# tlepoint/fhe.rs

Measured on NVIDIA H100. Metric: bfv_ct_mul_relin_per_sec_n32768_14x62bit, higher is better.
Workload: dtype u64

## Files before the change

### fhe_rs_b200/csrc/capi.cu

```cuda
#include <algorithm>
#include <atomic>
#include <cstring>
#include <map>
#include <memory>
#include <mutex>
#include <string>
#include <vector>

#include "../../include/fhe_b200.h"
#include "engine.hpp"
#include "host/precompute.hpp"

using namespace fhe_b200;

namespace {

thread_local std::string g_last_error;

struct ScalerData {
  ScalerTablesH h;
  ScalerDev dev;
};

struct LevelData {
// ... 334 lines not shown
    FHE_CUDA(cudaEventRecord(ev[ns], user));
    for (u32 i = 0; i < ns; i++) FHE_CUDA(cudaStreamWaitEvent(par->side[i], ev[ns], 0));
  }
  template <class F>
  void run(F&& body) {
    u32 k = 0;
    for (u32 c0 = 0; c0 < count; c0 += chunk, k++) body(c0, std::min(chunk, count - c0), ns > 1 ? par->side[k % ns] : user);
    join();
  }
  void join() {
    if (ns < 2 || joined) return;
    joined = true;
    for (u32 i = 0; i < ns; i++)
      if (cudaEventRecord(ev[i], par->side[i]) == cudaSuccess) cudaStreamWaitEvent(user, ev[i], 0);
  }
  ~ChunkRunner() {
    join();
    for (cudaEvent_t e : ev)
      if (e) cudaEventDestroy(e);
  }
  bool joined = false;
};

void check_same(const fhe_b200_batch* a, const fhe_b200_batch* b) {
  if (a->par != b->par) throw FheError(FHE_B200_CONTEXT_MISMATCH, "ParameterMismatch: batches use different parameters");
  if (a->level != b->level) throw FheError(FHE_B200_INVALID_LEVEL, "InvalidLevel: operands are at different levels");
  if (a->mul_basis != b->mul_basis || a->limbs != b->limbs)
    throw FheError(FHE_B200_CONTEXT_MISMATCH, "PolynomialContextMismatch");
}
void need_repr(const fhe_b200_batch* b, int repr) {
  if (b->repr != repr) throw FheError(FHE_B200_INVALID_REPRESENTATION, "IncorrectRepresentation");
}
const RowIds& ids_of(const fhe_b200_batch* b) {
  const LevelData& lv = b->par->level(b->level);
  return b->mul_basis ? lv.mul_ids : lv.ctx_ids;
}

void key_switch_core(const fhe_b200_params* par, const fhe_b200_ksk* k, const u64* c2, u32 cts, const u64* base0,
                     const u64* base1, u64* out0, u64* out1, u32 out_ct_rows, Workspace& ws, cudaStream_t st) {
  const LevelData& kl = par->level(k->ksk_level);
  const u32 L = k->n_dig, Lk = k->Lk;
  u64* inter = ws.words(((size_t)cts * L * Lk) << par->logn);
  bool adjacent = false;
  if (k->log_base) {
    u64* dig = ws.words(((size_t)cts * L) << par->logn);
    launch_decompose(c2, dig, cts, L, k->log_base, par->logn, st);
    launch_ntt(dig, inter, cts * L, kl.ctx_ids, par->d_limbs, par->logn, false, 1, false, st, true);
  } else {
  u64 qmax = 0, qmin = ~0ull;
  for (u32 i = 0; i < L; i++) qmax = std::max(qmax, par->moduli[i]);
  for (u32 j = 0; j < Lk; j++) qmin = std::min(qmin, par->moduli[j]);
  const bool reduce = qmax > 4 * qmin - 1 || qmin < (1ull << 8);
  adjacent = Lk > 1 && ntt_uses_tma(cts * L * Lk, kl.ctx_ids, par->logn, Lk, c2, inter);
  launch_ntt(c2, inter, cts * L * Lk, kl.ctx_ids, par->d_limbs, par->logn, false, Lk, reduce, st, true, adjacent, L);
  }
  launch_ksmac(inter, k->k0, k->k1, base0, base1, out0, out1, cts, L, Lk, out_ct_rows, kl.ctx_ids, par->d_limbs,
               par->logn, st, adjacent);
}

void key_switch_apply(const fhe_b200_params* par, const fhe_b200_ksk* k, const u64* c2, u32 cts, u64* out,
                      int base_mode, u64* base, Workspace& ws, cudaStream_t st) {
  const LevelData& cl = par->level(k->ct_level);
  const u32 L = cl.L, Lk = k->Lk, logn = par->logn;
  const size_t row = (size_t)1 << logn;
  if (Lk == L) {
    const u64* b0 = base_mode == 1 ? out : base_mode == 2 ? base : nullptr;
    const u64* b1 = base_mode == 1 ? out + L * row : nullptr;
    key_switch_core(par, k, c2, cts, b0, b1, out, out + L * row, 2 * L, ws, st);
    return;
  }
  u64* cur = ws.words((size_t)cts * 2 * Lk * row);
  key_switch_core(par, k, c2, cts, nullptr, nullptr, cur, cur + Lk * row, 2 * Lk, ws, st);
  const LevelData& kl = par->level(k->ksk_level);
  launch_ntt(cur, cur, cts * 2 * Lk, kl.ctx_ids, par->d_limbs, logn, true, 1, false, st);
  for (u32 lv = k->ksk_level; lv < k->ct_level; lv++) {
    const LevelData& from = par->level(lv);
    u64* nxt = ws.words((size_t)cts * 2 * (from.L - 1) * row);
    launch_switch_down(from.sd, cur, nxt, cts * 2, from.L, from.ctx_ids, par->d_limbs, logn, st);
    cur = nxt;
  }
  launch_ntt(cur, cur, cts * 2 * L, cl.ctx_ids, par->d_limbs, logn, false, 1, false, st);
  if (base_mode == 1) {
    launch_ew(EW_ADD, out, cur, (size_t)cts * 2 * L, cl.ctx_ids, par->d_limbs, logn, st);
  } else {
    FHE_CUDA(cudaMemcpyAsync(out, cur, (size_t)cts * 2 * L * row * sizeof(u64), cudaMemcpyDeviceToDevice, st));
    if (base_mode == 2) {
      FHE_CUDA(cudaMemset2DAsync(base + L * row, 2 * L * row * sizeof(u64), 0, L * row * sizeof(u64), cts, st));
      launch_ew(EW_ADD, out, base, (size_t)cts * 2 * L, cl.ctx_ids, par->d_limbs, logn, st);
    }
  }
}

void mul_core(const fhe_b200_params* par, const LevelData& lv, const u64* a, const u64* b, u32 cts, u64* out0,
              u64* out1, int split, Workspace& ws, cudaStream_t st) {
  const u32 L = lv.L, E = lv.E, K = lv.K, logn = par->logn;
  const size_t row = (size_t)1 << logn;
  u64* A_l = ws.words((size_t)cts * 2 * L * row);
  u64* A_r = ws.words((size_t)cts * 2 * L * row);
  u64* X_l = ws.words((size_t)cts * 2 * E * row);
  u64* X_r = ws.words((size_t)cts * 2 * E * row);
  u64* T = ws.words((size_t)cts * 3 * K * row);
  RowIds ext_ids;
  std::memset(&ext_ids, 0, sizeof(ext_ids));
  ext_ids.limbs_per_poly = E;
  for (u32 j = 0; j < E; j++) ext_ids.ids[j] = lv.mul_ids.ids[L + j];
  launch_ntt(a, A_l, cts * 2 * L, lv.ctx_ids, par->d_limbs, logn, true, 1, false, st);
// ... 985 lines not shown
```

### fhe_rs_b200/csrc/engine.hpp

```cpp
#pragma once
#include <atomic>
#include <cuda_runtime.h>

#include "ntt.cuh"

namespace fhe_b200 {

extern std::atomic<unsigned long long> g_launches;

struct CudaFail {
  cudaError_t err;
  const char* what;
};
#define FHE_CUDA(x)                                         \
  do {                                                      \
    cudaError_t e__ = (x);                                  \
    if (e__ != cudaSuccess) throw CudaFail{e__, #x};        \
  } while (0)

void ensure_dynamic_smem(const void* kernel, size_t bytes);

struct RowIds {
  u32 limbs_per_poly;
  unsigned short ids[kMaxPos];
};

void launch_ntt(const u64* in, u64* out, u32 n_rows, const RowIds& ids, const LimbDev* limbs, u32 logn,
                bool inverse, u32 in_div, bool reduce_on_load, cudaStream_t st, bool lazy_out = false,
                bool digit_adjacent = false, u32 n_dig = 1);

bool launch_tensor_inverse_ntt(const u64* a, const u64* b, const u64* xa, const u64* xb, u64* T, u32 cts, u32 L, u32 K,
                               const RowIds& mul_ids, const LimbDev* limbs, u32 logn, cudaStream_t st);

enum EwOp { EW_ADD = 0, EW_SUB = 1, EW_NEG = 2 };
void launch_ew(EwOp op, u64* a, const u64* b, size_t n_rows, const RowIds& ids, const LimbDev* limbs, u32 logn,
               cudaStream_t st);

void launch_mul_plain(u64* a, const u64* pt, u32 cts, u32 parts, u32 n_pt, const RowIds& ids, const LimbDev* limbs,
                      u32 logn, cudaStream_t st, u32 op = 0);

void launch_dot(const u64* ct, const u64* pt, u64* out, u32 groups, u32 n_terms, u32 parts, u32 ct_count,
                u32 pt_count, const RowIds& ids, const LimbDev* limbs, u32 logn, cudaStream_t st);

void launch_tensor(const u64* a, const u64* b, const u64* xa, const u64* xb, u64* out, u32 cts, u32 L, u32 nca,
                   u32 ncb, u32 K, const RowIds& mul_ids, const LimbDev* limbs, u32 logn, cudaStream_t st);

void launch_tensor_nm(const u64* a, const u64* b, const u64* xa, const u64* xb, u64* out, u32 cts, u32 L, u32 E, u32 na,
                      u32 nb, const RowIds& mul_ids, const LimbDev* limbs, u32 logn, cudaStream_t st);

struct ScalerDev {
  u32 n_from, n_to, is_one, shift;
  u64 tg_lo, tg_hi;
  u32 tg_sign;
  u32 all_solinas;
  const u64* gamma;
  const u64* omega;
  const u64* to_lo;
  const u64* to_hi;
  const unsigned char* to_sign;
  const unsigned char* to_order;
  u32 n_pos, n_terms;
  const u64* tgar_lo;
  const u64* tgar_hi;
  unsigned short to_ids[kMaxPos];
};
void launch_scale(const ScalerDev& S, const LimbDev* limbs, const u64* in, u64* out0, u64* out1, u32 polys,
                  u32 out_rows_per_poly, u32 start, u32 n_out, int split3, u32 logn, cudaStream_t st);

void launch_ksmac(const u64* inter, const u64* k0, const u64* k1, const u64* base0, const u64* base1, u64* out0,
                  u64* out1, u32 cts, u32 n_dig, u32 Lk, u32 out_ct_rows, const RowIds& ids, const LimbDev* limbs,
                  u32 logn, cudaStream_t st, bool adjacent = false);

bool ntt_uses_tma(u32 n_rows, const RowIds& ids, u32 logn, u32 in_div, const u64* in, const u64* out);

void launch_decompose(const u64* in, u64* out, size_t polys, u32 n_dig, u32 log_base, u32 logn, cudaStream_t st);

void launch_gather(const u64* in, u64* out, size_t n_rows, const int* perm, u32 logn, cudaStream_t st);
void launch_substitute_power(const u64* in, u64* out, size_t n_rows, u32 exponent, const RowIds& ids,
                             const LimbDev* limbs, u32 logn, cudaStream_t st);

struct SwitchDownDev {
  u64 q_last, q_last_half;
  const u64* half_mod;
  const u64* inv;
  const u64* inv_s;
};
void launch_switch_down(const SwitchDownDev& S, const u64* in, u64* out, u32 polys, u32 L, const RowIds& ids,
                        const LimbDev* limbs, u32 logn, cudaStream_t st);

struct PackDev {
  u32 limbs;
  unsigned char nbits[kMaxPos];
  u32 offs[kMaxPos];
  u32 poly_bytes;
};
void launch_pack(const PackDev& P, const u64* words, unsigned char* bytes, size_t n_rows, u32 logn, cudaStream_t st);
void launch_unpack(const PackDev& P, const unsigned char* bytes, u64* words, size_t n_rows, u32 logn, cudaStream_t st);

}
```

### fhe_rs_b200/csrc/ntt.cu

```cuda
#include <algorithm>
#include <cstdint>
#include <cstdlib>
#include <cstring>
#include <map>
#include <mutex>
#include <utility>

#include "engine.hpp"
#include "ntt_fast.cuh"
#include "ntt_tma.cuh"

namespace fhe_b200 {

std::atomic<unsigned long long> g_launches{0};

void ensure_dynamic_smem(const void* kernel, size_t bytes) {
  if (bytes <= 48 * 1024) return;
  static std::mutex mu;
  static std::map<std::pair<int, const void*>, size_t> granted;
  int dev = 0;
  FHE_CUDA(cudaGetDevice(&dev));
  std::lock_guard<std::mutex> g(mu);
  size_t& have = granted[std::make_pair(dev, kernel)];
  if (have >= bytes) return;
// ... 171 lines not shown
  g_launches++;
}

template <bool INV>
void run_tma_rows(const u64* in, u64 in_rows, u64* out, u64 out_rows, const NttTmaArgs& A, cudaStream_t st) {
  static const int v = tma_variant("FHE_B200_TMA_ROWS", 2);
  if (v == 2 && A.n_polys % 2 == 0 && !(A.digit_adjacent && A.n_dig % 2)) {
    run_tma_rows_pair<INV, 3, 3>(in, in_rows, out, out_rows, A, st);
    return;
  }
  if (v == 26) run_tma_rows_v<INV, 2, 6>(in, in_rows, out, out_rows, A, st);
  else run_tma_rows_v<INV, 4, 4>(in, in_rows, out, out_rows, A, st);
}
template <int LOGP, bool INV, int STAGES, int MINB>
void run_tma_cols_v(const u64* in, u64 in_rows, u64* out, u64 out_rows, NttTmaArgs A, cudaStream_t st) {
  using Cfg = ColsCfg<LOGP, STAGES>;
  const CUtensorMap mi = cols_map(in, in_rows, A.logn, Cfg::BOX_ROWS), mo = cols_map(out, out_rows, A.logn, Cfg::BOX_ROWS);
  A.tiles_per_row = 4;
  A.tiles_total = A.lpp * 4 * A.n_polys;
  const u32 grid = std::min<u64>(A.tiles_total, (u64)sm_count() * MINB);
  if (!INV && A.reduce_on_load) {
    auto k = ntt_tma_cols_kernel<LOGP, INV, STAGES, MINB, !INV>;
    ensure_dynamic_smem((const void*)k, Cfg::SMEM);
    k<<<grid, Cfg::NT + 32, Cfg::SMEM, st>>>(mi, mo, A);
  } else {
    auto k = ntt_tma_cols_kernel<LOGP, INV, STAGES, MINB, false>;
    ensure_dynamic_smem((const void*)k, Cfg::SMEM);
    k<<<grid, Cfg::NT + 32, Cfg::SMEM, st>>>(mi, mo, A);
  }
  g_launches++;
}
template <int LOGP, bool INV>
void run_tma_cols(const u64* in, u64 in_rows, u64* out, u64 out_rows, const NttTmaArgs& A, cudaStream_t st) {
  static const int v = tma_variant("FHE_B200_TMA_COLS", 3);
  if (LOGP == 9) {
    if (v == 2) run_tma_cols_v<9, INV, 2, 1>(in, in_rows, out, out_rows, A, st);
    else run_tma_cols_v<9, INV, 3, 1>(in, in_rows, out, out_rows, A, st);
  } else if (LOGP == 8) {
    if (v == 2) run_tma_cols_v<8, INV, 2, 3>(in, in_rows, out, out_rows, A, st);
    else run_tma_cols_v<8, INV, 3, 2>(in, in_rows, out, out_rows, A, st);
  } else {
    if (v == 2) run_tma_cols_v<7, INV, 2, 6>(in, in_rows, out, out_rows, A, st);
    else run_tma_cols_v<7, INV, 3, 4>(in, in_rows, out, out_rows, A, st);
  }
}
template <bool INV>
void run_tma_cols_for(const u64* in, u64 in_rows, u64* out, u64 out_rows, const NttTmaArgs& A, cudaStream_t st) {
  switch (A.logn - 6) {
    case 7: run_tma_cols<7, INV>(in, in_rows, out, out_rows, A, st); break;
    case 8: run_tma_cols<8, INV>(in, in_rows, out, out_rows, A, st); break;
    case 9: run_tma_cols<9, INV>(in, in_rows, out, out_rows, A, st); break;
    default: throw TmaFail{};
  }
}

bool launch_ntt_tma(const u64* in, u64* out, u32 n_rows, const RowIds& ids, const LimbDev* limbs, u32 logn, bool inverse,
                    u32 in_div, bool reduce_on_load, cudaStream_t st, bool lazy_out, bool digit_adjacent, u32 n_dig) {
  const u32 lpp = ids.limbs_per_poly;
  if (logn < 13 || logn > 15 || !tensor_map_encoder()) return false;
  if (n_rows % lpp != 0 || (in_div != 1 && in_div != lpp)) return false;
  if (digit_adjacent && ((n_rows / lpp) % n_dig != 0 || n_dig == 0)) return false;
  if ((reinterpret_cast<uintptr_t>(in) | reinterpret_cast<uintptr_t>(out)) & 127) return false;
  NttTmaArgs A;
  std::memset(&A, 0, sizeof(A));
  A.limbs = limbs;
  A.n_polys = n_rows / lpp;
  A.lpp = lpp;
  A.logn = logn;
  A.digit_adjacent = digit_adjacent ? 1 : 0;
  A.n_dig = digit_adjacent ? n_dig : 1;
  for (int i = 0; i < kMaxPos; i++) A.ids[i] = ids.ids[i];
  const u64 in_rows = in_div == 1 ? n_rows : n_rows / lpp;
  try {
    NttTmaArgs first = A, second = A;
    first.in_bcast = in_div != 1;
    if (!inverse) {
      first.reduce_on_load = reduce_on_load;
      second.lazy_out = lazy_out;
      run_tma_cols_for<false>(in, in_rows, out, n_rows, first, st);
      run_tma_rows<false>(out, n_rows, out, n_rows, second, st);
    } else {
      if (reduce_on_load || in_div != 1) return false;
      run_tma_rows<true>(in, in_rows, out, n_rows, first, st);
      run_tma_cols_for<true>(out, n_rows, out, n_rows, second, st);
    }
  } catch (const TmaFail&) {
    return false;
  }
  return true;
}

template <int STAGES, int MINB>
void run_tensor_rows(const CUtensorMap& ma, const CUtensorMap& mb, const CUtensorMap& mxa, const CUtensorMap& mxb,
                     const CUtensorMap& mo, TensorRowsArgs A, cudaStream_t st) {
  using Cfg = TensorRowsCfg<kRowsRlog, STAGES>;
  auto k = ntt_tma_tensor_rows_kernel<kRowsRlog, STAGES, MINB>;
  ensure_dynamic_smem((const void*)k, Cfg::SMEM);
  const u32 grid = std::min<u64>(A.items_total, (u64)sm_count() * MINB);
  k<<<grid, Cfg::NT + 32, Cfg::SMEM, st>>>(ma, mb, mxa, mxb, mo, A);
  g_launches++;
}

bool launch_tensor_intt_tma(const u64* a, const u64* b, const u64* xa, const u64* xb, u64* T, u32 cts, u32 L, u32 K,
                            const RowIds& mul_ids, const LimbDev* limbs, u32 logn, cudaStream_t st) {
  constexpr u32 R = 1u << kRowsRlog;
  const u32 E = K - L;
  try {
    const CUtensorMap ma = rows_map(a, (u64)cts * 2 * L, logn, 4 * R), mb = rows_map(b, (u64)cts * 2 * L, logn, 4 * R);
    const CUtensorMap mxa = rows_map(xa, (u64)cts * 2 * E, logn, 4 * R), mxb = rows_map(xb, (u64)cts * 2 * E, logn, 4 * R);
    const CUtensorMap mo = rows_map(T, (u64)cts * 3 * K, logn, 4 * R);
    TensorRowsArgs A;
    std::memset(&A, 0, sizeof(A));
    A.limbs = limbs; A.cts = cts; A.L = L; A.K = K; A.logn = logn;
    A.tiles_per_row = (1u << (logn - 6)) / R;
    A.items_total = K * A.tiles_per_row * cts;
    for (int i = 0; i < kMaxPos; i++) A.ids[i] = mul_ids.ids[i];
    static const int v = tma_variant("FHE_B200_TENSOR_V", 22);
    if (v == 13) run_tensor_rows<1, 3>(ma, mb, mxa, mxb, mo, A, st);
    else if (v == 14) run_tensor_rows<1, 4>(ma, mb, mxa, mxb, mo, A, st);
    else run_tensor_rows<2, 2>(ma, mb, mxa, mxb, mo, A, st);
    NttTmaArgs C;
    std::memset(&C, 0, sizeof(C));
    C.limbs = limbs; C.n_polys = cts * 3; C.lpp = K; C.logn = logn; C.n_dig = 1;
    for (int i = 0; i < kMaxPos; i++) C.ids[i] = mul_ids.ids[i];
    run_tma_cols_for<true>(T, (u64)cts * 3 * K, T, (u64)cts * 3 * K, C, st);
  } catch (const TmaFail&) {
    return false;
  }
  return true;
}

int tma_mode() {
  static const int mode = [] {
    const char* e = getenv("FHE_B200_NTT");
    if (getenv("FHE_B200_GENERIC_NTT") || getenv("FHE_B200_SOLINAS_NTT")) return 0;
    if (e && !strcmp(e, "fast")) return 0;
    if (e && !strcmp(e, "tma")) return 2;
    return 1;
  }();
  return mode;
}

}

bool ntt_uses_tma(u32 n_rows, const RowIds& ids, u32 logn, u32 in_div, const u64* in, const u64* out) {
  const u32 lpp = ids.limbs_per_poly;
  if (!tma_mode() || logn < 13 || logn > 15 || !tensor_map_encoder()) return false;
  if (n_rows % lpp != 0 || (in_div != 1 && in_div != lpp)) return false;
  if ((reinterpret_cast<uintptr_t>(in) | reinterpret_cast<uintptr_t>(out)) & 127) return false;
  return tma_mode() == 2 || n_rows / lpp >= 8;
}

bool launch_tensor_inverse_ntt(const u64* a, const u64* b, const u64* xa, const u64* xb, u64* T, u32 cts, u32 L, u32 K,
                               const RowIds& mul_ids, const LimbDev* limbs, u32 logn, cudaStream_t st) {
  static const bool off = getenv("FHE_B200_NO_TENSOR_FUSION") != nullptr;
  if (off || K <= L || !ntt_uses_tma(cts * 3 * K, mul_ids, logn, 1, T, T)) return false;
  if ((reinterpret_cast<uintptr_t>(a) | reinterpret_cast<uintptr_t>(b) | reinterpret_cast<uintptr_t>(xa) |
       reinterpret_cast<uintptr_t>(xb)) & 127)
    return false;
  return launch_tensor_intt_tma(a, b, xa, xb, T, cts, L, K, mul_ids, limbs, logn, st);
}

void launch_ntt(const u64* in, u64* out, u32 n_rows, const RowIds& ids, const LimbDev* limbs, u32 logn,
                bool inverse, u32 in_div, bool reduce_on_load, cudaStream_t st, bool lazy_out, bool digit_adjacent,
                u32 n_dig) {
  if (n_rows == 0) return;
  NttArgs a;
  a.in = in;
  a.out = out;
  a.limbs = limbs;
  a.n_rows = n_rows;
  a.limbs_per_poly = ids.limbs_per_poly;
  a.in_div = in_div;
  a.reduce_on_load = reduce_on_load ? 1 : 0;
  a.lazy_out = (lazy_out && !inverse) ? 1 : 0;
  a.logn = logn;
  for (int i = 0; i < kMaxPos; i++) a.ids[i] = ids.ids[i];
  if (logn <= 12) {
    a.logn1 = 0;
    if (inverse) run_single<true>(a, st); else run_single<false>(a, st);
    return;
  }
  a.logn1 = logn - 6;
  NttArgs second = a;
  second.in = out;
  second.in_div = 1;
  second.reduce_on_load = 0;
  if (ntt_uses_tma(n_rows, ids, logn, in_div, in, out) &&
      launch_ntt_tma(in, out, n_rows, ids, limbs, logn, inverse, in_div, reduce_on_load, st, lazy_out, digit_adjacent,
                     n_dig))
    return;
  if (digit_adjacent) throw CudaFail{cudaErrorNotSupported, "digit-adjacent NTT output needs the TMA kernels"};
  static const bool generic = getenv("FHE_B200_GENERIC_NTT") != nullptr || getenv("FHE_B200_SOLINAS_NTT") != nullptr;
  if (generic) {
    if (!inverse) {
      run_cols_for<false>(a, st);
      run_rows<6, 6, false>(second, st);
    } else {
      run_rows<6, 6, true>(a, st);
      run_cols_for<true>(second, st);
    }
    return;
  }
  static const int rows_tlog = getenv("FHE_B200_ROWS_TLOG") ? atoi(getenv("FHE_B200_ROWS_TLOG")) : 10;
  static const int cols_tlog = getenv("FHE_B200_COLS_TLOG") ? atoi(getenv("FHE_B200_COLS_TLOG")) : 11;
  auto rows = [&](const NttArgs& x, bool inv) {
    if (rows_tlog == 10) { if (inv) run_fast<6, false, true, 10>(x, st); else run_fast<6, false, false, 10>(x, st); }
    else { if (inv) run_fast<6, false, true>(x, st); else run_fast<6, false, false>(x, st); }
  };
  auto cols = [&](const NttArgs& x, bool inv) {
    if (cols_tlog == 11 && x.logn1 <= 9) { if (inv) run_fast_cols_for<true, 11>(x, st); else run_fast_cols_for<false, 11>(x, st); }
    else { if (inv) run_fast_cols_for<true>(x, st); else run_fast_cols_for<false>(x, st); }
  };
// ... 11 lines not shown
```

### fhe_rs_b200/csrc/ntt_tma.cuh

```cuda
#pragma once
#include <cuda.h>

#include "ntt.cuh"

namespace fhe_b200 {

struct NttTmaArgs {
  const LimbDev* limbs;
  u32 n_polys;
  u32 lpp;
  u32 in_bcast;
  u32 digit_adjacent;
  u32 n_dig;
  u32 reduce_on_load;
  u32 lazy_out;
  u32 logn;
  u32 tiles_per_row;
  u32 tiles_total;
  unsigned short ids[kMaxPos];
};

namespace tma {

__device__ __forceinline__ u32 smem_u32(const void* p) { return (u32)__cvta_generic_to_shared(p); }
__device__ __forceinline__ void mbar_init(u32 bar, u32 count) {
  asm volatile("mbarrier.init.shared::cta.b64 [%0], %1;" ::"r"(bar), "r"(count) : "memory");
}
__device__ __forceinline__ void mbar_expect_tx(u32 bar, u32 bytes) {
  asm volatile("mbarrier.arrive.expect_tx.shared::cta.b64 _, [%0], %1;" ::"r"(bar), "r"(bytes) : "memory");
}
__device__ __forceinline__ void mbar_arrive(u32 bar) {
  asm volatile("mbarrier.arrive.shared::cta.b64 _, [%0];" ::"r"(bar) : "memory");
}
__device__ __forceinline__ u32 mbar_try_wait(u32 bar, u32 parity, u32 ns) {
  u32 ok;
  asm volatile(
      "{\n\t"
      ".reg .pred p;\n\t"
      "mbarrier.try_wait.parity.shared::cta.b64 p, [%1], %2, %3;\n\t"
      "selp.u32 %0, 1, 0, p;\n\t"
      "}"
      : "=r"(ok)
      : "r"(bar), "r"(parity), "r"(ns)
      : "memory");
  return ok;
}
__device__ __forceinline__ void mbar_wait(u32 bar, u32 parity) {
  u32 tries = 0;
  while (!mbar_try_wait(bar, parity, 100000u)) {
    if (++tries > 4000000u) __trap();
  }
}
__device__ __forceinline__ void fence_proxy_async() { asm volatile("fence.proxy.async.shared::cta;" ::: "memory"); }
__device__ __forceinline__ void bulk_commit() { asm volatile("cp.async.bulk.commit_group;" ::: "memory"); }
template <int N>
__device__ __forceinline__ void bulk_wait_read() {
  asm volatile("cp.async.bulk.wait_group.read %0;" ::"n"(N) : "memory");
}
__device__ __forceinline__ void bulk_wait_all() { asm volatile("cp.async.bulk.wait_group 0;" ::: "memory"); }
template <int NT>
__device__ __forceinline__ void consumer_sync() {
  asm volatile("bar.sync 1, %0;" ::"n"(NT) : "memory");
}

__device__ __forceinline__ void load_2d(u32 dst, const CUtensorMap* tm, u32 c0, u32 c1, u32 bar) {
  asm volatile(
      "cp.async.bulk.tensor.2d.shared::cluster.global.tile.mbarrier::complete_tx::bytes [%0], [%1, {%2, %3}], [%4];"
      ::"r"(dst), "l"(tm), "r"(c0), "r"(c1), "r"(bar)
      : "memory");
}
__device__ __forceinline__ void store_2d(const CUtensorMap* tm, u32 c0, u32 c1, u32 src) {
  asm volatile("cp.async.bulk.tensor.2d.global.shared::cta.tile.bulk_group [%0, {%1, %2}], [%3];" ::"l"(tm), "r"(c0),
               "r"(c1), "r"(src)
               : "memory");
}
__device__ __forceinline__ void load_3d(u32 dst, const CUtensorMap* tm, u32 c0, u32 c1, u32 c2, u32 bar) {
  asm volatile(
      "cp.async.bulk.tensor.3d.shared::cluster.global.tile.mbarrier::complete_tx::bytes [%0], [%1, {%2, %3, %4}], "
      "[%5];" ::"r"(dst),
      "l"(tm), "r"(c0), "r"(c1), "r"(c2), "r"(bar)
      : "memory");
}
__device__ __forceinline__ void store_3d(const CUtensorMap* tm, u32 c0, u32 c1, u32 c2, u32 src) {
  asm volatile("cp.async.bulk.tensor.3d.global.shared::cta.tile.bulk_group [%0, {%1, %2, %3}], [%4];" ::"l"(tm),
               "r"(c0), "r"(c1), "r"(c2), "r"(src)
               : "memory");
}
__device__ __forceinline__ void prefetch_map(const CUtensorMap* tm) {
  asm volatile("prefetch.tensormap [%0];" ::"l"(tm) : "memory");
}

__device__ __forceinline__ u64 lds64(u32 a) {
  u64 v;
  asm volatile("ld.shared.u64 %0, [%1];" : "=l"(v) : "r"(a));
  return v;
}
__device__ __forceinline__ void sts64(u32 a, u64 v) { asm volatile("st.shared.u64 [%0], %1;" ::"r"(a), "l"(v) : "memory"); }
__device__ __forceinline__ ulonglong2 lds128(u32 a) {
  ulonglong2 v;
  asm volatile("ld.shared.v2.u64 {%0, %1}, [%2];" : "=l"(v.x), "=l"(v.y) : "r"(a));
  return v;
}
__device__ __forceinline__ void sts128(u32 a, u64 x, u64 y) {
  asm volatile("st.shared.v2.u64 [%0], {%1, %2};" ::"r"(a), "l"(x), "l"(y) : "memory");
}

template <int NS>
__device__ __forceinline__ void fwd_stages(u64* v, const ulonglong2* tw, u64 p, u64 p2) {
  constexpr int R = 1 << NS;
#pragma unroll
  for (int u = 0; u < NS; u++) {
    const int half = R >> (u + 1);
#pragma unroll
    for (int m = 0; m < (1 << u); m++) {
      const ulonglong2 w = tw[(1 << u) - 1 + m];
#pragma unroll
      for (int e = 0; e < half; e++) {
        const int jj = m * 2 * half + e;
        bf_fwd<false>(v[jj], v[jj + half], w.x, w.y, p, p2, 0);
      }
    }
  }
}
struct LastStage {
  u64 ninv, ninv_s, zn, zn_s;
};
template <int NS, typename LS>
__device__ __forceinline__ void inv_stages(u64* v, const ulonglong2* tz, u64 p, u64 p2, bool last, const LS& L) {
  constexpr int R = 1 << NS;
#pragma unroll
  for (int u = NS - 1; u >= 0; u--) {
    const int half = R >> (u + 1);
    if (u == 0 && last) {
#pragma unroll
      for (int e = 0; e < half; e++) {
        const u64 a = v[e], b2 = v[e + half];
        v[e] = csub(mul_shoup_lazy(a + b2, L.ninv, L.ninv_s, p), p);
        v[e + half] = csub(mul_shoup_lazy(p2 + a - b2, L.zn, L.zn_s, p), p);
      }
    } else {
#pragma unroll
      for (int m = 0; m < (1 << u); m++) {
        const ulonglong2 z = tz[(1 << u) - 1 + m];
#pragma unroll
        for (int e = 0; e < half; e++) {
          const int jj = m * 2 * half + e;
          bf_inv<false>(v[jj], v[jj + half], z.x, z.y, p, p2, 0);
        }
      }
    }
  }
}

struct TileWalk {
  u32 jt, p, n_polys;
  __device__ __forceinline__ void init(u32 idx, u32 np) {
    n_polys = np;
    jt = idx / np;
    p = idx - jt * np;
  }
  __device__ __forceinline__ bool next() {
    if (++p == n_polys) {
      p = 0;
      jt++;
      return true;
    }
    return false;
  }
};

__device__ __forceinline__ u32 out_row_of(const NttTmaArgs& A, u32 p, u32 j) {
  if (A.digit_adjacent) {
// ... 549 lines not shown
      Acc192 sx, sy;
      sx.clear();
      sy.clear();
      sx.mac(a0.x, b1.x);
      sx.mac(a1.x, b0.x);
      sy.mac(a0.y, b1.y);
      sy.mac(a1.y, b0.y);
      const u64 c1x = sx.reduce_lazy(M), c1y = sy.reduce_lazy(M);
      sts128(o, c0x, c0y);
      sts128(o + 2 * TILE_BYTES, c1x, c1y);
      sts128(o + TILE_BYTES, c2x, c2y);
    }
    u64 v[8];
    ulonglong2 tw[7];
    tw[0] = lds128(tw3);
    tw[1] = lds128(tw4);
    tw[2] = lds128(tw4 + 16 * 8 * R);
#pragma unroll
    for (int m = 0; m < 4; m++) tw[3 + m] = lds128(tw5 + 16 * 8 * R * m);
#pragma unroll 1
    for (u32 t = 0; t < 3; t++) {
      const u32 tb = buf + t * TILE_BYTES;
#pragma unroll
      for (int k = 0; k < 4; k++) {
        const ulonglong2 q = lds128(tb + off1[k]);
        v[2 * k] = q.x;
        v[2 * k + 1] = q.y;
      }
      inv_stages<3>(v, tw, p, p2, false, M);
#pragma unroll
      for (int k = 0; k < 4; k++) sts128(tb + off1[k], v[2 * k], v[2 * k + 1]);
    }
    consumer_sync<NT>();
    tw[0] = lds128(tw0);
    tw[1] = lds128(tw1);
    tw[2] = lds128(tw1 + 16);
#pragma unroll
    for (int m = 0; m < 4; m++) tw[3 + m] = lds128(tw2 + 16 * m);
#pragma unroll 1
    for (u32 t = 0; t < 3; t++) {
      const u32 tb = buf + t * TILE_BYTES;
#pragma unroll
      for (int e = 0; e < 8; e++) v[e] = lds64(tb + off0[e]);
      inv_stages<3>(v, tw, p, p2, false, M);
#pragma unroll
      for (int e = 0; e < 8; e++) sts64(tb + off0[e], v[e]);
    }
    fence_proxy_async();
    mbar_arrive(bar_done + 8 * s);
    fresh = w.next();
  }
}

template <int LOGP, int STAGES>
struct ColsCfg {
  static constexpr u32 P = 1u << LOGP;
  static constexpr u32 NT = P;
  static constexpr u32 TILE_BYTES = P * 128;
  static constexpr u32 BOX_ROWS = P < 256 ? P : 256;
  static constexpr u32 BOXES = P / BOX_ROWS;
  static constexpr u32 SMEM = STAGES * TILE_BYTES + P * 16 + 2 * STAGES * 8 + 1024;
  static constexpr int NR = (LOGP + 2) / 3;
  static constexpr int REM = LOGP - 3 * (NR - 1);
};

template <int LOGP, bool INV, int NS, int T, bool REDUCE, bool ROLL = false>
__device__ __forceinline__ void cols_round(u32 buf, u32 tw_base, u64 p, u64 p2, const tma::LastStage& L, u64 bhi, u64 blo) {
  using namespace tma;
  constexpr int t = T;
  constexpr u32 NT = 1u << LOGP;
  constexpr int R = 1 << NS;
  constexpr u32 UNITS = (1u << (LOGP + 4 - NS)) / NT;
  constexpr int logstride = LOGP - t - NS;
  constexpr u32 stride_bytes = 128u << logstride;
  constexpr bool HI = (LOGP - 4) >= logstride;
  constexpr u32 D_AHI = HI ? (1u << (LOGP - 4 - logstride)) : 0;
  constexpr u32 D_ADDR = (HI ? (D_AHI << (LOGP - t)) : (1u << (LOGP - 4))) * 128;
  const u32 bcol = threadIdx.x & 15, rest = threadIdx.x >> 4;
  const u32 a_lo = rest & ((1u << logstride) - 1);
  u32 a_hi = rest >> logstride;
  u32 addr = buf + ((a_hi << (LOGP - t)) + a_lo) * 128 + bcol * 8;
#pragma unroll(ROLL ? 1 : 8)
  for (u32 q = 0; q < UNITS; q++) {
    u64 v[R];
#pragma unroll
    for (int e = 0; e < R; e++) {
      v[e] = lds64(addr + e * stride_bytes);
      if (REDUCE) v[e] = barrett64(v[e], p, bhi, blo);
    }
    ulonglong2 tw[R - 1];
#pragma unroll
    for (int u = 0; u < NS; u++) {
      const int tl = t + u;
      if (INV && tl == 0) continue;
      const u32 idx = (INV ? ((1u << LOGP) - (2u << tl)) : (1u << tl)) + (a_hi << u);
#pragma unroll
      for (int m = 0; m < (1 << u); m++) tw[(1 << u) - 1 + m] = lds128(tw_base + 16 * (idx + m));
    }
    if (!INV) fwd_stages<NS>(v, tw, p, p2);
    else inv_stages<NS>(v, tw, p, p2, t == 0, L);
#pragma unroll
    for (int e = 0; e < R; e++) sts64(addr + e * stride_bytes, v[e]);
    addr += D_ADDR;
    a_hi += D_AHI;
  }
}

template <int LOGP, bool INV, int STAGES, int MINB, bool REDUCE, bool ROLL = false>
__global__ void __launch_bounds__(ColsCfg<LOGP, STAGES>::NT + 32, MINB)
    ntt_tma_cols_kernel(const __grid_constant__ CUtensorMap tm_in, const __grid_constant__ CUtensorMap tm_out,
                        const NttTmaArgs A) {
  using namespace tma;
  using Cfg = ColsCfg<LOGP, STAGES>;
  constexpr u32 NT = Cfg::NT, TILE_BYTES = Cfg::TILE_BYTES, P = Cfg::P;
  constexpr int NR = Cfg::NR, REM = Cfg::REM;
  extern __shared__ unsigned char smem_raw[];
  const u32 base = (smem_u32(smem_raw) + 1023u) & ~1023u;
  const u32 tw_base = base + STAGES * TILE_BYTES;
  const u32 bar_full = tw_base + P * 16;
  const u32 bar_done = bar_full + STAGES * 8;

  if (threadIdx.x == 0) {
#pragma unroll
    for (int s = 0; s < STAGES; s++) {
      mbar_init(bar_full + 8 * s, 1);
      mbar_init(bar_done + 8 * s, NT);
    }
    asm volatile("fence.mbarrier_init.release.cluster;" ::: "memory");
  }
  __syncthreads();

  const u32 lo = (u32)(((u64)A.tiles_total * blockIdx.x) / gridDim.x);
  const u32 hi = (u32)(((u64)A.tiles_total * (blockIdx.x + 1)) / gridDim.x);
  const u32 n = hi - lo;

  if (threadIdx.x >= NT) {
    if (threadIdx.x != NT) return;
    prefetch_map(&tm_in);
    prefetch_map(&tm_out);
    TileWalk wl, ws;
    wl.init(lo, A.n_polys);
    ws.init(lo, A.n_polys);
    u32 loaded = 0;
    auto load_next = [&]() {
      const u32 s = loaded % STAGES;
      const u32 j = wl.jt / A.tiles_per_row, tau = wl.jt - j * A.tiles_per_row;
      const u32 row = A.in_bcast ? wl.p : out_row_of(A, wl.p, j);
      mbar_expect_tx(bar_full + 8 * s, TILE_BYTES);
#pragma unroll
      for (u32 h = 0; h < Cfg::BOXES; h++)
        load_3d(base + s * TILE_BYTES + h * Cfg::BOX_ROWS * 128, &tm_in, tau * 16, h * Cfg::BOX_ROWS, row,
                bar_full + 8 * s);
      wl.next();
      loaded++;
    };
    while (loaded < n && loaded < (u32)STAGES) load_next();
    for (u32 i = 0; i < n; i++) {
      const u32 s = i % STAGES;
      mbar_wait(bar_done + 8 * s, (i / STAGES) & 1);
      const u32 j = ws.jt / A.tiles_per_row, tau = ws.jt - j * A.tiles_per_row;
      const u32 row = out_row_of(A, ws.p, j);
#pragma unroll
      for (u32 h = 0; h < Cfg::BOXES; h++)
        store_3d(&tm_out, tau * 16, h * Cfg::BOX_ROWS, row, base + s * TILE_BYTES + h * Cfg::BOX_ROWS * 128);
      bulk_commit();
      ws.next();
      if (loaded < n) {
        bulk_wait_read<0>();
        load_next();
      }
    }
    bulk_wait_all();
    return;
  }

  const u32 tid = threadIdx.x;
  TileWalk w;
  w.init(lo, A.n_polys);
  u32 cur_j = 0xffffffffu;
  const LimbDev* Lp = A.limbs;
  u64 p = 0, p2 = 0, bhi = 0, blo = 0;
  LastStage ls = {0, 0, 0, 0};
  for (u32 i = 0; i < n; i++) {
    const u32 j = w.jt / A.tiles_per_row;
    if (j != cur_j) {
      Lp = A.limbs + A.ids[j];
      p = Lp->p;
      p2 = Lp->p2;
      if (INV) ls = LastStage{Lp->ninv, Lp->ninv_s, Lp->zn, Lp->zn_s};
      if (REDUCE) {
        bhi = Lp->bhi;
        blo = Lp->blo;
      }
      const ulonglong2* tab = INV ? Lp->zi + ((1u << A.logn) - P) : Lp->om;
      if (cur_j != 0xffffffffu) consumer_sync<NT>();
      for (u32 k = tid; k < P; k += NT) {
        const ulonglong2 v = __ldg(tab + k);
        sts128(tw_base + 16 * k, v.x, v.y);
      }
      consumer_sync<NT>();
      cur_j = j;
    }
    const u32 s = i % STAGES;
    const u32 buf = base + s * TILE_BYTES;
    mbar_wait(bar_full + 8 * s, (i / STAGES) & 1);
    if (!INV) {
#pragma unroll
      for (int r = 0; r < NR; r++) {
        if (r == 0) cols_round<LOGP, false, 3, 0, REDUCE, ROLL>(buf, tw_base, p, p2, ls, bhi, blo);
        else if (r == 1 && NR > 2) cols_round<LOGP, false, 3, 3, false, ROLL>(buf, tw_base, p, p2, ls, bhi, blo);
        else cols_round<LOGP, false, REM, 3 * (NR - 1), false, ROLL>(buf, tw_base, p, p2, ls, bhi, blo);
        if (r < NR - 1) consumer_sync<NT>();
      }
    } else {
#pragma unroll
      for (int r = NR - 1; r >= 0; r--) {
        if (r == 0) cols_round<LOGP, true, 3, 0, false, ROLL>(buf, tw_base, p, p2, ls, bhi, blo);
        else if (r == 1 && NR > 2) cols_round<LOGP, true, 3, 3, false, ROLL>(buf, tw_base, p, p2, ls, bhi, blo);
        else cols_round<LOGP, true, REM, 3 * (NR - 1), false, ROLL>(buf, tw_base, p, p2, ls, bhi, blo);
        if (r > 0) consumer_sync<NT>();
      }
    }
    fence_proxy_async();
    mbar_arrive(bar_done + 8 * s);
    w.next();
  }
}

}
```

Before: 3546.

## Fuse key-switch row NTT stage with key MAC in a TMA kernel

Adds a TMA-pipelined kernel that runs the second (row) pass of the forward NTT on the digit tiles and, in the same pass, multiply-accumulates them against the relinearization key tiles. It writes the key-switch output directly, so the intermediate NTT output is never written and read back by a separate ksmac kernel. The column-pass NTT also gains a limb-inner tile walk order for broadcast inputs, which is intended to improve reuse of each input row across limbs. The fused kernel needs a large shared-memory allocation per block, which can lower occupancy, and it falls back to the old path when its preconditions fail.

```diff
diff --git a/fhe_rs_b200/csrc/capi.cu b/fhe_rs_b200/csrc/capi.cu
--- a/fhe_rs_b200/csrc/capi.cu
+++ b/fhe_rs_b200/csrc/capi.cu
@@ -410,6 +410,14 @@
   for (u32 j = 0; j < Lk; j++) qmin = std::min(qmin, par->moduli[j]);
   const bool reduce = qmax > 4 * qmin - 1 || qmin < (1ull << 8);
   adjacent = Lk > 1 && ntt_uses_tma(cts * L * Lk, kl.ctx_ids, par->logn, Lk, c2, inter);
+  static const bool fused = [] {
+    const char* e = getenv("FHE_B200_KSMAC");
+    return !e || (strcmp(e, "tma") && strcmp(e, "classic"));
+  }();
+  if (adjacent && fused &&
+      launch_key_switch_tma(c2, inter, k->k0, k->k1, base0, base1, out0, out1, cts, L, Lk, out_ct_rows, kl.ctx_ids,
+                            par->d_limbs, par->logn, reduce, st))
+    return;
   launch_ntt(c2, inter, cts * L * Lk, kl.ctx_ids, par->d_limbs, par->logn, false, Lk, reduce, st, true, adjacent, L);
   }
   launch_ksmac(inter, k->k0, k->k1, base0, base1, out0, out1, cts, L, Lk, out_ct_rows, kl.ctx_ids, par->d_limbs,
diff --git a/fhe_rs_b200/csrc/engine.hpp b/fhe_rs_b200/csrc/engine.hpp
--- a/fhe_rs_b200/csrc/engine.hpp
+++ b/fhe_rs_b200/csrc/engine.hpp
@@ -73,6 +73,10 @@
 
 bool ntt_uses_tma(u32 n_rows, const RowIds& ids, u32 logn, u32 in_div, const u64* in, const u64* out);
 
+bool launch_key_switch_tma(const u64* c2, u64* inter, const u64* k0, const u64* k1, const u64* base0,
+                           const u64* base1, u64* out0, u64* out1, u32 cts, u32 n_dig, u32 Lk, u32 out_ct_rows,
+                           const RowIds& ids, const LimbDev* limbs, u32 logn, bool reduce, cudaStream_t st);
+
 void launch_decompose(const u64* in, u64* out, size_t polys, u32 n_dig, u32 log_base, u32 logn, cudaStream_t st);
 
 void launch_gather(const u64* in, u64* out, size_t n_rows, const int* perm, u32 logn, cudaStream_t st);
diff --git a/fhe_rs_b200/csrc/ntt.cu b/fhe_rs_b200/csrc/ntt.cu
--- a/fhe_rs_b200/csrc/ntt.cu
+++ b/fhe_rs_b200/csrc/ntt.cu
@@ -247,6 +247,14 @@
     case 9: run_tma_cols<9, INV>(in, in_rows, out, out_rows, A, st); break;
     default: throw TmaFail{};
   }
+}
+
+bool bcast_limb_inner() {
+  static const bool v = [] {
+    const char* e = getenv("FHE_B200_BCAST_WALK");
+    return !(e && !strcmp(e, "limb_major"));
+  }();
+  return v;
 }
 
 bool launch_ntt_tma(const u64* in, u64* out, u32 n_rows, const RowIds& ids, const LimbDev* limbs, u32 logn, bool inverse,
@@ -269,6 +277,7 @@
   try {
     NttTmaArgs first = A, second = A;
     first.in_bcast = in_div != 1;
+    first.limb_inner = first.in_bcast && bcast_limb_inner();
     if (!inverse) {
       first.reduce_on_load = reduce_on_load;
       second.lazy_out = lazy_out;
@@ -325,6 +334,33 @@
   return true;
 }
 
+template <int STAGES>
+void run_ks_rows_mac(const CUtensorMap& mi, const CUtensorMap& m0, const CUtensorMap& m1, const KsRowsArgs& A,
+                     cudaStream_t st) {
+  using Cfg = KsRowsCfg<STAGES>;
+  auto k = ks_rows_mac_tma_kernel<STAGES, 3>;
+  const size_t smem = Cfg::smem(A.n_dig);
+  ensure_dynamic_smem((const void*)k, smem);
+  int per_sm = 0;
+  FHE_CUDA(cudaOccupancyMaxActiveBlocksPerMultiprocessor(&per_sm, (const void*)k, Cfg::NT + 32, smem));
+  const u32 grid = (u32)std::min<u64>(A.items_total, (u64)sm_count() * std::max(per_sm, 1));
+  k<<<grid, Cfg::NT + 32, smem, st>>>(mi, m0, m1, A);
+  g_launches++;
+}
+
+CUtensorMap key_map(const u64* base, u64 rows, u32 logn, u32 box_cols, u32 box_rows) {
+  CUtensorMap m;
+  const cuuint64_t gdim[2] = {(cuuint64_t)1 << logn, rows};
+  const cuuint64_t gstride[1] = {(cuuint64_t)8 << logn};
+  const cuuint32_t box[2] = {box_cols, box_rows};
+  const cuuint32_t es[2] = {1, 1};
+  if (tensor_map_encoder()(&m, CU_TENSOR_MAP_DATA_TYPE_UINT64, 2, (void*)base, gdim, gstride, box, es,
+                           CU_TENSOR_MAP_INTERLEAVE_NONE, CU_TENSOR_MAP_SWIZZLE_NONE, CU_TENSOR_MAP_L2_PROMOTION_L2_128B,
+                           CU_TENSOR_MAP_FLOAT_OOB_FILL_NONE) != CUDA_SUCCESS)
+    throw TmaFail{};
+  return m;
+}
+
 int tma_mode() {
   static const int mode = [] {
     const char* e = getenv("FHE_B200_NTT");
@@ -354,6 +390,51 @@
        reinterpret_cast<uintptr_t>(xb)) & 127)
     return false;
   return launch_tensor_intt_tma(a, b, xa, xb, T, cts, L, K, mul_ids, limbs, logn, st);
+}
+
+bool launch_key_switch_tma(const u64* c2, u64* inter, const u64* k0, const u64* k1, const u64* base0,
+                           const u64* base1, u64* out0, u64* out1, u32 cts, u32 n_dig, u32 Lk, u32 out_ct_rows,
+                           const RowIds& ids, const LimbDev* limbs, u32 logn, bool reduce, cudaStream_t st) {
+  static const int stages = tma_variant("FHE_B200_KS_STAGES", 2) >= 3 ? 3 : 2;
+  using Cfg = KsRowsCfg<2>;
+  const u32 n_rows = cts * n_dig * Lk;
+  if (logn < 13 || logn > 15 || !tensor_map_encoder() || ids.limbs_per_poly != Lk || n_dig == 0 || n_dig > 256)
+    return false;
+  if ((reinterpret_cast<uintptr_t>(c2) | reinterpret_cast<uintptr_t>(inter) | reinterpret_cast<uintptr_t>(k0) |
+       reinterpret_cast<uintptr_t>(k1)) & 127)
+    return false;
+  if ((stages == 3 ? KsRowsCfg<3>::smem(n_dig) : Cfg::smem(n_dig)) > 227 * 1024) return false;
+  try {
+    const CUtensorMap mi = rows_map(inter, n_rows, logn, 4 * Cfg::R);
+    const CUtensorMap m0 = key_map(k0, (u64)Lk * n_dig, logn, Cfg::TC, n_dig);
+    const CUtensorMap m1 = key_map(k1, (u64)Lk * n_dig, logn, Cfg::TC, n_dig);
+    NttTmaArgs C;
+    std::memset(&C, 0, sizeof(C));
+    C.limbs = limbs;
+    C.n_polys = cts * n_dig;
+    C.lpp = Lk;
+    C.in_bcast = 1;
+    C.limb_inner = bcast_limb_inner();
+    C.digit_adjacent = 1;
+    C.n_dig = n_dig;
+    C.reduce_on_load = reduce ? 1 : 0;
+    C.logn = logn;
+    for (int i = 0; i < kMaxPos; i++) C.ids[i] = ids.ids[i];
+    run_tma_cols_for<false>(c2, (u64)cts * n_dig, inter, n_rows, C, st);
+    KsRowsArgs A;
+    std::memset(&A, 0, sizeof(A));
+    A.limbs = limbs;
+    A.base0 = base0; A.base1 = base1; A.out0 = out0; A.out1 = out1;
+    A.cts = cts; A.n_dig = n_dig; A.Lk = Lk; A.out_ct_rows = out_ct_rows; A.logn = logn;
+    A.tiles_per_row = (1u << logn) / Cfg::TC;
+    A.items_total = Lk * A.tiles_per_row * cts;
+    for (int i = 0; i < kMaxPos; i++) A.ids[i] = ids.ids[i];
+    if (stages == 3) run_ks_rows_mac<3>(mi, m0, m1, A, st);
+    else run_ks_rows_mac<2>(mi, m0, m1, A, st);
+  } catch (const TmaFail&) {
+    return false;
+  }
+  return true;
 }
 
 void launch_ntt(const u64* in, u64* out, u32 n_rows, const RowIds& ids, const LimbDev* limbs, u32 logn,
diff --git a/fhe_rs_b200/csrc/ntt_tma.cuh b/fhe_rs_b200/csrc/ntt_tma.cuh
--- a/fhe_rs_b200/csrc/ntt_tma.cuh
+++ b/fhe_rs_b200/csrc/ntt_tma.cuh
@@ -17,6 +17,7 @@
   u32 logn;
   u32 tiles_per_row;
   u32 tiles_total;
+  u32 limb_inner;
   unsigned short ids[kMaxPos];
 };
 
@@ -118,6 +119,24 @@
       for (int e = 0; e < half; e++) {
         const int jj = m * 2 * half + e;
         bf_fwd<false>(v[jj], v[jj + half], w.x, w.y, p, p2, 0);
+      }
+    }
+  }
+}
+template <class TW>
+__device__ __forceinline__ void fwd_stages3_staged(u64* v, u64 p, u64 p2, const TW& tw) {
+#pragma unroll
+  for (int u = 0; u < 3; u++) {
+    const int half = 8 >> (u + 1);
+    ulonglong2 w[4];
+#pragma unroll
+    for (int m = 0; m < (1 << u); m++) w[m] = tw(u, m);
+#pragma unroll
+    for (int m = 0; m < (1 << u); m++) {
+#pragma unroll
+      for (int e = 0; e < half; e++) {
+        const int jj = m * 2 * half + e;
+        bf_fwd<false>(v[jj], v[jj + half], w[m].x, w[m].y, p, p2, 0);
       }
     }
   }
@@ -773,6 +792,179 @@
   }
 }
 
+struct KsRowsArgs {
+  const LimbDev* limbs;
+  const u64 *base0, *base1;
+  u64 *out0, *out1;
+  u32 cts, n_dig, Lk, out_ct_rows, logn;
+  u32 tiles_per_row;
+  u32 items_total;
+  unsigned short ids[kMaxPos];
+};
+
+template <int STAGES>
+struct KsRowsCfg {
+  static constexpr u32 R = 2;
+  static constexpr u32 TC = 64 * R;
+  static constexpr u32 TILE_BYTES = 512 * R;
+  static constexpr u32 GROUPS = 16;
+  static constexpr u32 NT = GROUPS * 8 * R;
+  static constexpr u32 TW_PAIRS = 63 * R;
+  static constexpr size_t smem(u32 nd) {
+    return (size_t)STAGES * nd * TILE_BYTES + 2 * (size_t)nd * TC * 8 + TW_PAIRS * 16 + 2 * STAGES * 8 + 8 + 1024;
+  }
+};
+
+template <int STAGES, int MINB>
+__global__ void __launch_bounds__(KsRowsCfg<STAGES>::NT + 32, MINB)
+    ks_rows_mac_tma_kernel(const __grid_constant__ CUtensorMap tm_in, const __grid_constant__ CUtensorMap tm_k0,
+                           const __grid_constant__ CUtensorMap tm_k1, const KsRowsArgs A) {
+  using namespace tma;
+  using Cfg = KsRowsCfg<STAGES>;
+  constexpr u32 R = Cfg::R, TC = Cfg::TC, NT = Cfg::NT, TILE_BYTES = Cfg::TILE_BYTES, GROUPS = Cfg::GROUPS;
+  extern __shared__ unsigned char smem_raw[];
+  const u32 nd = A.n_dig;
+  const u32 base = (smem_u32(smem_raw) + 1023u) & ~1023u;
+  const u32 stage_bytes = nd * TILE_BYTES;
+  const u32 k0_base = base + STAGES * stage_bytes;
+  const u32 k1_base = k0_base + nd * TC * 8;
+  const u32 tw_base = k1_base + nd * TC * 8;
+  const u32 bar_full = tw_base + Cfg::TW_PAIRS * 16;
+  const u32 bar_done = bar_full + STAGES * 8;
+  const u32 bar_key = bar_done + STAGES * 8;
+
+  if (threadIdx.x == 0) {
+#pragma unroll
+    for (int s = 0; s < STAGES; s++) {
+      mbar_init(bar_full + 8 * s, 1);
+      mbar_init(bar_done + 8 * s, NT);
+    }
+    mbar_init(bar_key, 1);
+    asm volatile("fence.mbarrier_init.release.cluster;" ::: "memory");
+  }
+  __syncthreads();
+
+  const u32 lo = (u32)(((u64)A.items_total * blockIdx.x) / gridDim.x);
+  const u32 hi = (u32)(((u64)A.items_total * (blockIdx.x + 1)) / gridDim.x);
+  const u32 n = hi - lo;
+  const u32 box_rows_per_row = (1u << A.logn) >> 4;
+
+  if (threadIdx.x >= NT) {
+    if (threadIdx.x != NT) return;
+    prefetch_map(&tm_in);
+    TileWalk wl;
+    wl.init(lo, A.cts);
+    for (u32 i = 0; i < n; i++) {
+      const u32 s = i % STAGES;
+      if (i >= (u32)STAGES) mbar_wait(bar_done + 8 * s, (i / STAGES - 1) & 1);
+      const u32 j = wl.jt / A.tiles_per_row, tau = wl.jt - j * A.tiles_per_row;
+      const u32 row0 = (wl.p * A.Lk + j) * nd;
+      mbar_expect_tx(bar_full + 8 * s, stage_bytes);
+      for (u32 d = 0; d < nd; d++)
+        load_2d(base + s * stage_bytes + d * TILE_BYTES, &tm_in, 0, (row0 + d) * box_rows_per_row + tau * (4 * R),
+                bar_full + 8 * s);
+      wl.next();
+    }
+    return;
+  }
+
+  const u32 tid = threadIdx.x;
+  const u32 g = tid >> 4, lt = tid & 15;
+  const u32 hmask = 0xffffu << (tid & 16);
+  const u32 x = lt & 7, b = lt >> 3;
+  const u32 off0 = ((4 * b) << 7) | ((((x >> 1) & 7) ^ (4 * b)) << 4) | ((x & 1) << 3);
+  const u32 off1 = ((4 * b + (x >> 1)) << 7) | (((4 * (x & 1)) ^ (4 * b + (x >> 1))) << 4);
+  auto x0 = [](int e) -> u32 { return ((u32)(e >> 1) << 7) | ((u32)((e >> 1) ^ (4 * (e & 1))) << 4); };
+  const u32 tw0 = tw_base + 16 * (b);
+  const u32 tw1 = tw_base + 16 * (R * 1 + (b << 1));
+  const u32 tw2 = tw_base + 16 * (R * 3 + (b << 2));
+  const u32 tw3 = tw_base + 16 * (R * 7 + lt);
+  const u32 tw4 = tw_base + 16 * (R * 15 + lt);
+  const u32 tw5 = tw_base + 16 * (R * 31 + lt);
+  const u32 c = tid & (TC - 1), o = tid / TC;
+  const u32 offc = ((c >> 4) << 7) | ((((c >> 1) & 7) ^ ((c >> 4) & 7)) << 4) | ((c & 1) << 3);
+  const u32 key_c = (o ? k1_base : k0_base) + 8 * c;
+  const u64* bsrc = o ? A.base1 : A.base0;
+  u64* dst = o ? A.out1 : A.out0;
+
+  TileWalk w;
+  w.init(lo, A.cts);
+  bool fresh = true;
+  u32 key_phase = 0;
+  const LimbDev* Mp = A.limbs;
+  u64 p = 0, p2 = 0;
+  const u32 logn1 = A.logn - 6;
+  for (u32 i = 0; i < n; i++) {
+    const u32 j = w.jt / A.tiles_per_row, tau = w.jt - j * A.tiles_per_row;
+    const bool new_keys = fresh;
+    if (fresh) {
+      Mp = A.limbs + A.ids[j];
+      p = Mp->p;
+      p2 = Mp->p2;
+      if (i) consumer_sync<NT>();
+      if (tid == 0) {
+        mbar_expect_tx(bar_key, 2 * nd * TC * 8);
+        load_2d(k0_base, &tm_k0, tau * TC, j * nd, bar_key);
+        load_2d(k1_base, &tm_k1, tau * TC, j * nd, bar_key);
+      }
+      const u32 row0 = tau * R;
+#pragma unroll
+      for (int tl = 0; tl < 6; tl++) {
+        const u32 s = logn1 + tl;
+        const u32 g0 = (1u << s) + (row0 << tl);
+        if (tid < (R << tl)) {
+          const ulonglong2 v = __ldg(Mp->om + g0 + tid);
+          const u32 k = tid;
+          const u32 dst_pair = tl < 3 ? k : (k & ((1u << (tl >= 3 ? tl - 3 : 0)) - 1)) * (8 * R) + (k >> (tl >= 3 ? tl - 3 : 0));
+          sts128(tw_base + 16 * (R * ((1u << tl) - 1) + dst_pair), v.x, v.y);
+        }
+      }
+      consumer_sync<NT>();
+    }
+    const size_t oi = (((size_t)w.p * A.out_ct_rows + j) << A.logn) + tau * TC + c;
+    const u64 bv = bsrc ? bsrc[oi] : 0;
+    const u32 s = i % STAGES;
+    const u32 ring = base + s * stage_bytes;
+    mbar_wait(bar_full + 8 * s, (i / STAGES) & 1);
+    for (u32 d = g; d < nd; d += GROUPS) {
+      const u32 a0 = ring + d * TILE_BYTES + off0, a1 = ring + d * TILE_BYTES + off1;
+      u64 v[8];
+#pragma unroll
+      for (int e = 0; e < 8; e++) v[e] = lds64(a0 ^ x0(e));
+      fwd_stages3_staged(v, p, p2, [&](int u, int m) {
+        return lds128(u == 0 ? tw0 : u == 1 ? tw1 + 16 * m : tw2 + 16 * m);
+      });
+#pragma unroll
+      for (int e = 0; e < 8; e++) sts64(a0 ^ x0(e), v[e]);
+      __syncwarp(hmask);
+#pragma unroll
+      for (int k = 0; k < 4; k++) {
+        const ulonglong2 t = lds128(a1 ^ (k << 4));
+        v[2 * k] = t.x;
+        v[2 * k + 1] = t.y;
+      }
+      fwd_stages3_staged(v, p, p2, [&](int u, int m) {
+        return lds128(u == 0 ? tw3 : u == 1 ? tw4 + 16 * 8 * R * m : tw5 + 16 * 8 * R * m);
+      });
+#pragma unroll
+      for (int k = 0; k < 4; k++) sts128(a1 ^ (k << 4), v[2 * k], v[2 * k + 1]);
+    }
+    if (new_keys) {
+      mbar_wait(bar_key, key_phase);
+      key_phase ^= 1;
+    }
+    consumer_sync<NT>();
+    Acc192 acc;
+    acc.clear();
+#pragma unroll 2
+    for (u32 d = 0; d < nd; d++) acc.mac(lds64(ring + d * TILE_BYTES + offc), lds64(key_c + d * TC * 8));
+    acc.add64(bv);
+    dst[oi] = acc.reduce(*Mp);
+    mbar_arrive(bar_done + 8 * s);
+    fresh = w.next();
+  }
+}
+
 template <int LOGP, int STAGES>
 struct ColsCfg {
   static constexpr u32 P = 1u << LOGP;
@@ -827,6 +1019,20 @@
   }
 }
 
+__device__ __forceinline__ void cols_tile(const NttTmaArgs& A, u32 idx, u32& j, u32& tau, u32& p) {
+  if (A.limb_inner) {
+    const u32 r = idx / A.lpp;
+    j = idx - r * A.lpp;
+    tau = r / A.n_polys;
+    p = r - tau * A.n_polys;
+  } else {
+    const u32 jt = idx / A.n_polys;
+    p = idx - jt * A.n_polys;
+    j = jt / A.tiles_per_row;
+    tau = jt - j * A.tiles_per_row;
+  }
+}
+
 template <int LOGP, bool INV, int STAGES, int MINB, bool REDUCE, bool ROLL = false>
 __global__ void __launch_bounds__(ColsCfg<LOGP, STAGES>::NT + 32, MINB)
     ntt_tma_cols_kernel(const __grid_constant__ CUtensorMap tm_in, const __grid_constant__ CUtensorMap tm_out,
@@ -859,33 +1065,30 @@
     if (threadIdx.x != NT) return;
     prefetch_map(&tm_in);
     prefetch_map(&tm_out);
-    TileWalk wl, ws;
-    wl.init(lo, A.n_polys);
-    ws.init(lo, A.n_polys);
     u32 loaded = 0;
     auto load_next = [&]() {
       const u32 s = loaded % STAGES;
-      const u32 j = wl.jt / A.tiles_per_row, tau = wl.jt - j * A.tiles_per_row;
-      const u32 row = A.in_bcast ? wl.p : out_row_of(A, wl.p, j);
+      u32 j, tau, pp;
+      cols_tile(A, lo + loaded, j, tau, pp);
+      const u32 row = A.in_bcast ? pp : out_row_of(A, pp, j);
       mbar_expect_tx(bar_full + 8 * s, TILE_BYTES);
 #pragma unroll
       for (u32 h = 0; h < Cfg::BOXES; h++)
         load_3d(base + s * TILE_BYTES + h * Cfg::BOX_ROWS * 128, &tm_in, tau * 16, h * Cfg::BOX_ROWS, row,
                 bar_full + 8 * s);
-      wl.next();
       loaded++;
     };
     while (loaded < n && loaded < (u32)STAGES) load_next();
     for (u32 i = 0; i < n; i++) {
       const u32 s = i % STAGES;
       mbar_wait(bar_done + 8 * s, (i / STAGES) & 1);
-      const u32 j = ws.jt / A.tiles_per_row, tau = ws.jt - j * A.tiles_per_row;
-      const u32 row = out_row_of(A, ws.p, j);
+      u32 j, tau, pp;
+      cols_tile(A, lo + i, j, tau, pp);
+      const u32 row = out_row_of(A, pp, j);
 #pragma unroll
       for (u32 h = 0; h < Cfg::BOXES; h++)
         store_3d(&tm_out, tau * 16, h * Cfg::BOX_ROWS, row, base + s * TILE_BYTES + h * Cfg::BOX_ROWS * 128);
       bulk_commit();
-      ws.next();
       if (loaded < n) {
         bulk_wait_read<0>();
         load_next();
@@ -896,14 +1099,13 @@
   }
 
   const u32 tid = threadIdx.x;
-  TileWalk w;
-  w.init(lo, A.n_polys);
   u32 cur_j = 0xffffffffu;
   const LimbDev* Lp = A.limbs;
   u64 p = 0, p2 = 0, bhi = 0, blo = 0;
   LastStage ls = {0, 0, 0, 0};
   for (u32 i = 0; i < n; i++) {
-    const u32 j = w.jt / A.tiles_per_row;
+    u32 j, tau_unused, p_unused;
+    cols_tile(A, lo + i, j, tau_unused, p_unused);
     if (j != cur_j) {
       Lp = A.limbs + A.ids[j];
       p = Lp->p;
@@ -944,8 +1146,7 @@
     }
     fence_proxy_async();
     mbar_arrive(bar_done + 8 * s);
-    w.next();
-  }
-}
-
-}
+  }
+}
+
+}
diff --git a/profiles/kernel_shares.py b/profiles/kernel_shares.py
--- /dev/null
+++ b/profiles/kernel_shares.py
@@ -0,0 +1,87 @@
+import argparse
+import json
+import os
+import subprocess
+import sys
+
+ROOT = os.path.dirname(os.path.dirname(os.path.abspath(__file__)))
+sys.path.insert(0, ROOT)
+import numpy as np
+import torch
+from torch.profiler import ProfilerActivity, profile
+
+import fhe_rs_b200 as F
+from bench import DEGREE, N_MODULI, PLAINTEXT, fill_uniform
+
+
+def card():
+    try:
+        q = subprocess.run(["nvidia-smi", "--query-gpu=name,power.limit", "--format=csv,noheader,nounits", "-i", "0"],
+                           capture_output=True, text=True, timeout=30).stdout.strip().split(", ")
+        return {"gpu": q[0], "power_limit_w": float(q[1])}
+    except Exception:
+        return {"gpu": torch.cuda.get_device_name(0), "power_limit_w": None}
+
+
+def short(name):
+    name = name.replace("(anonymous namespace)::", "").replace("void ", "").replace("fhe_b200::", "")
+    return name.split("(")[0] or name
+
+
+def main():
+    ap = argparse.ArgumentParser()
+    ap.add_argument("what", nargs="?", default="mulrelin", choices=["mulrelin", "rotate"])
+    ap.add_argument("batch", nargs="?", type=int, default=256)
+    ap.add_argument("--steps", type=int, default=2)
+    ap.add_argument("--json", help="also write the table as JSON")
+    a = ap.parse_args()
+
+    par = F.BfvParameters(DEGREE, PLAINTEXT, moduli_sizes=[62] * N_MODULI, device=0)
+    moduli = par.moduli()
+    A = F.Ciphertext(par, a.batch, 2)
+    fill_uniform(torch, A, moduli, 1)
+    rng = np.random.default_rng(7)
+    kc = np.zeros((2, N_MODULI, N_MODULI, DEGREE), np.uint64)
+    for i, q in enumerate(moduli):
+        kc[:, :, i, :] = rng.integers(0, q, size=(2, N_MODULI, DEGREE), dtype=np.uint64)
+    if a.what == "mulrelin":
+        B = F.Ciphertext(par, a.batch, 2)
+        fill_uniform(torch, B, moduli, 2)
+        m = F.Multiplicator.default(F.RelinearizationKey.from_arrays(par, kc[0], kc[1]))
+        op = lambda: m.multiply(A, B)
+    else:
+        gk = F.GaloisKey.from_arrays(par, 3, kc[0], kc[1])
+        op = lambda: gk.relinearize(A)
+    op().sync()
+    torch.cuda.synchronize()
+    with profile(activities=[ProfilerActivity.CUDA]) as prof:
+        for _ in range(a.steps):
+            out = op()
+        out.sync()
+        torch.cuda.synchronize()
+
+    per = {}
+    for ev in prof.events():
+        if ev.device_type != torch.autograd.DeviceType.CUDA:
+            continue
+        k = short(ev.name)
+        t, c = per.get(k, (0.0, 0))
+        per[k] = (t + ev.time_range.elapsed_us(), c + 1)
+    total = sum(t for t, _ in per.values())
+    rows = sorted(((k, t, c) for k, (t, c) in per.items()), key=lambda r: -r[1])
+    info = card()
+    print("%s, power limit %s W; %s batch %d, %d steps; summed kernel time %.2f ms per step"
+          % (info["gpu"], info["power_limit_w"], a.what, a.batch, a.steps, total / 1e3 / a.steps))
+    print("%8s %6s %7s  %s" % ("ms/step", "share", "launch", "kernel"))
+    for k, t, c in rows:
+        print("%8.3f %5.1f%% %7.1f  %s" % (t / 1e3 / a.steps, 100.0 * t / total, c / a.steps, k))
+    if a.json:
+        with open(a.json, "w") as f:
+            json.dump({**info, "what": a.what, "batch": a.batch, "steps": a.steps,
+                       "kernel_ms_per_step": total / 1e3 / a.steps,
+                       "kernels": [{"name": k, "ms_per_step": t / 1e3 / a.steps, "share": t / total,
+                                    "launches_per_step": c / a.steps} for k, t, c in rows]}, f, indent=1)
+
+
+if __name__ == "__main__":
+    main()
```

Result: faster. 3683, median of 6 (+3.9%).
